# f-dangel/vivit

Hardware: AMD Instinct MI355X
Metric: GGN eigenpairs/sec (Gram build + symeig), MLP 784-512-10, batch=4096 (higher is better)
Workload: dtype f32

## Files before the change

### vivit_amd/csrc/sy2sb.hip

```cpp
#include <cstdlib>

#include "common.h"
#include "device_utils.h"
#include "eig_internal.h"

namespace vivit {

constexpr int SNB = 64;
constexpr int QT = 128;
constexpr int SGRP = 8;

__global__ __launch_bounds__(256) void sb_panel_load_kernel(const float *__restrict__ A, int64_t lda, int64_t j0, int64_t mp,
                                                            float *__restrict__ pan) {
  const int64_t idx = (int64_t)blockIdx.x * 256 + threadIdx.x;
  if (idx >= mp * SNB) return;
  const int64_t r = idx / SNB, c = idx - r * SNB;
  pan[idx] = A[(j0 + SNB + r) * lda + j0 + c];
}

__global__ __launch_bounds__(256) void sb_panel_load_row_kernel(const float *__restrict__ A, int64_t lda, int64_t j0, int64_t mp,
                                                                float *__restrict__ pan) {
  __shared__ float t[SNB][SNB + 1];
  const int64_t r0 = (int64_t)blockIdx.x * SNB;
  const int tid = threadIdx.x;
  for (int idx = tid; idx < SNB * SNB; idx += 256) {
    const int c = idx / SNB, rr = idx % SNB;
    t[c][rr] = r0 + rr < mp ? A[(j0 + c) * lda + j0 + SNB + r0 + rr] : 0.f;
  }
  __syncthreads();
  for (int idx = tid; idx < SNB * SNB; idx += 256) {
    const int rr = idx / SNB, c = idx % SNB;
    if (r0 + rr < mp) pan[(r0 + rr) * SNB + c] = t[c][rr];
  }
}

__global__ __launch_bounds__(256) void coef_gather_kernel(const float *__restrict__ S, int64_t lds_, int64_t g, int kp,
                                                          float *__restrict__ Coef) {
  const int idx = blockIdx.x * 256 + threadIdx.x;
  if (idx >= SNB * kp) return;
  const int k = idx / SNB, m = idx % SNB;
  Coef[(int64_t)m * kp + k] = S[(int64_t)k * lds_ + g + m];
}


__global__ __launch_bounds__(256) void qr_step_kernel(float *__restrict__ pan, int64_t mp, int c, int ncol, int nwg, QrPart pt,
                                                      float *__restrict__ vdst1, float *__restrict__ vdst2, int64_t lds_, int64_t gi0,
                                                      float *__restrict__ A, int64_t lda, int64_t j0,
                                                      float *__restrict__ tau1, float *__restrict__ betas) {
  __shared__ float tile[QT][SNB + 1];
  __shared__ float vs[QT], xs2[QT];
  __shared__ float zs[SNB];
  __shared__ float zq[4][SNB];
  __shared__ __attribute__((aligned(16))) float zq16[16][SNB];
  const int tid = threadIdx.x;
  const int64_t r0 = (int64_t)blockIdx.x * QT;
  constexpr int NTL = QT * (SNB / 4) / 256;
  float4 tl[NTL];
#pragma unroll
  for (int i = 0; i < NTL; ++i) {
    const int idx = tid + 256 * i;
    const int rl = idx / (SNB / 4), c4 = (idx - rl * (SNB / 4)) * 4;
    const int64_t r = r0 + rl;
    tl[i] = *reinterpret_cast<const float4 *>(pan + (r < mp ? r : 0) * SNB + c4);
  }
  const int par = c & 1;
  const float *uin = pt.u + (int64_t)par * nwg * SNB;
  const float *din = pt.diag + par * SNB;
  const int cq4 = tid & 15, q16 = tid >> 4;
  float4 pv[20];
#pragma unroll
  for (int i = 0; i < 20; ++i) {
    const int w = q16 + 16 * i;
    pv[i] = *reinterpret_cast<const float4 *>(uin + (int64_t)(w < nwg ? w : 0) * SNB + 4 * cq4);
  }
  const float din_c = din[c >= 0 ? c : 0], din_t = din[tid & (SNB - 1)];
  __builtin_amdgcn_sched_barrier(0);
#pragma unroll
  for (int i = 0; i < NTL; ++i) {
    const int idx = tid + 256 * i;
    const int rl = idx / (SNB / 4), c4 = (idx - rl * (SNB / 4)) * 4;
    const bool ok = r0 + rl < mp;
    tile[rl][c4 + 0] = ok ? tl[i].x : 0.f;
    tile[rl][c4 + 1] = ok ? tl[i].y : 0.f;
    tile[rl][c4 + 2] = ok ? tl[i].z : 0.f;
    tile[rl][c4 + 3] = ok ? tl[i].w : 0.f;
  }
  if (c >= 0) {
    {
      float4 acc = make_float4(0.f, 0.f, 0.f, 0.f);
#pragma unroll
      for (int i = 0; i < 20; ++i)
        if (q16 + 16 * i < nwg) { acc.x += pv[i].x; acc.y += pv[i].y; acc.z += pv[i].z; acc.w += pv[i].w; }
      for (int w0 = q16 + 16 * 20; w0 < nwg; w0 += 16 * 20) {
        float4 v[20];
#pragma unroll
        for (int i = 0; i < 20; ++i) {
          const int w = w0 + 16 * i;
          v[i] = *reinterpret_cast<const float4 *>(uin + (int64_t)(w < nwg ? w : 0) * SNB + 4 * cq4);
        }
#pragma unroll
        for (int i = 0; i < 20; ++i)
          if (w0 + 16 * i < nwg) { acc.x += v[i].x; acc.y += v[i].y; acc.z += v[i].z; acc.w += v[i].w; }
      }
      *reinterpret_cast<float4 *>(&zq16[q16][4 * cq4]) = acc;
    }
    __syncthreads();
    float ssq = 0.f;
#pragma unroll
    for (int g2 = 0; g2 < 16; ++g2) ssq += zq16[g2][c];
    const float alpha = din_c;
    float tau = 0.f, beta = alpha, scal = 0.f;
    if (ssq > 0.f) {
      beta = -copysignf(sqrt_nr(alpha * alpha + ssq), alpha);
      tau = (beta - alpha) * rcp_nr(beta);
      scal = rcp_nr(alpha - beta);
    }
    if (tid < SNB) {
      float u = 0.f;
#pragma unroll
      for (int g2 = 0; g2 < 16; ++g2) u += zq16[g2][tid];
      zs[tid] = tid > c ? tau * (din_t + scal * u) : 0.f;
    }
    if (tid < QT) {
      const int64_t r = r0 + tid;
      float v = 0.f;
      if (r < mp) {
        if (r == c) v = 1.f;
        else if (r > c) v = tile[tid][c] * scal;
        vdst1[(int64_t)c * lds_ + gi0 + r] = v;
        vdst2[(int64_t)c * lds_ + gi0 + r] = v;
        if (r >= c) A[(j0 + c) * lda + gi0 + r] = v;
      }
      vs[tid] = v;
    }
    if (blockIdx.x == 0 && tid == 0) { tau1[j0 + c] = tau; betas[c] = beta; }
  } else {
    if (tid < QT) vs[tid] = 0.f;
    if (tid < SNB) zs[tid] = 0.f;
  }
  __syncthreads();
  const int cn = c + 1;
  const bool has_next = cn < ncol;
  if (tid < QT) {
    const int64_t r = r0 + tid;
    xs2[tid] = (has_next && r > cn && r < mp) ? tile[tid][cn] - vs[tid] * zs[cn] : 0.f;
  }
  __syncthreads();
  {
    const int cc = tid & 63, q = tid >> 6;
    const float zc = zs[cc];
    float acc = 0.f;
#pragma unroll 8
    for (int i = 0; i < QT / 4; ++i) {
      const int rl = q + 4 * i;
      const float v = vs[rl];
      float x = tile[rl][cc];
      if (cc > c && v != 0.f) {
        x -= v * zc;
        tile[rl][cc] = x;
        if (r0 + rl < mp) pan[(r0 + rl) * SNB + cc] = x;
      }
      acc += xs2[rl] * x;
    }
    zq[q][cc] = acc;
  }
  if (!has_next) return;
  __syncthreads();
  {
    const int par = cn & 1;
    if (tid < SNB) pt.u[((int64_t)par * nwg + blockIdx.x) * SNB + tid] = (zq[0][tid] + zq[1][tid]) + (zq[2][tid] + zq[3][tid]);
    if (cn >= r0 && cn < r0 + QT && tid < SNB) pt.diag[par * SNB + tid] = tile[cn - r0][tid];
  }
}

constexpr int QP_WG = 32, QP_THREADS = 512;
struct QrPersistWs {
  float *ubuf;
  float *dbuf;
  int *counter;
  int *tmo;
  int attempt;
  int fault;
};

__device__ __forceinline__ float sel8(float a0, float a1, float a2, float a3, float a4, float a5, float a6, float a7, int j) {
  const float t0 = (j & 1) ? a1 : a0, t1 = (j & 1) ? a3 : a2, t2 = (j & 1) ? a5 : a4, t3 = (j & 1) ? a7 : a6;
  const float u0 = (j & 2) ? t1 : t0, u1 = (j & 2) ? t3 : t2;
  return (j & 4) ? u1 : u0;
}

template <int RI>
__global__ __launch_bounds__(QP_THREADS) void qr_persist_kernel(float *__restrict__ pan, int64_t mp, int ncol, QrPersistWs pw,
                                                                float *__restrict__ vdst1, float *__restrict__ vdst2, int64_t lds_,
                                                                int64_t gi0, float *__restrict__ A, int64_t lda, int64_t j0,
                                                                float *__restrict__ tau1, float *__restrict__ betas) {
  if ((blockIdx.x & 7) != 0) return;
  if (pw.attempt == 1 && __hip_atomic_load(pw.counter + 1, __ATOMIC_RELAXED, __HIP_MEMORY_SCOPE_AGENT) != PERSIST_ABORT) return;
  int *const cnt = pw.counter + 8 * pw.attempt;
  const int w = blockIdx.x >> 3;
  const int tid = threadIdx.x, lane = tid & 63, wave = tid >> 6;
  const int cg = tid & 7, rs = tid >> 3;
  constexpr int RW = 64 * RI;
  const int64_t rbase = (int64_t)w * RW;
  __shared__ float s_u[SNB], s_d[SNB], s_dn[SNB];
  __shared__ float s_red[QP_THREADS / 64][SNB];
  __shared__ float s_v[RW];
  __shared__ int s_flag[2];

  float x[RI][8];
#pragma unroll
  for (int i = 0; i < RI; ++i) {
    const int64_t r = rbase + rs + 64 * i;
    const float *src = pan + (r < mp ? r : 0) * SNB + 8 * cg;
    const float4 a = *reinterpret_cast<const float4 *>(src), b = *reinterpret_cast<const float4 *>(src + 4);
    const bool ok = r < mp;
    x[i][0] = ok ? a.x : 0.f; x[i][1] = ok ? a.y : 0.f; x[i][2] = ok ? a.z : 0.f; x[i][3] = ok ? a.w : 0.f;
    x[i][4] = ok ? b.x : 0.f; x[i][5] = ok ? b.y : 0.f; x[i][6] = ok ? b.z : 0.f; x[i][7] = ok ? b.w : 0.f;
  }
  if (tid == 0) {
    int xcc;
    __asm__ volatile("s_getreg_b32 %0, hwreg(HW_REG_XCC_ID)" : "=s"(xcc));
    __hip_atomic_store(pw.counter + 32 + w, xcc & 15, __ATOMIC_RELAXED, __HIP_MEMORY_SCOPE_AGENT);
    __asm__ volatile("s_waitcnt vmcnt(0)" ::: "memory");
    const bool go = persist_arrive(cnt, cnt + 1, QP_WG, ((pw.fault >> pw.attempt) & 1) ? 0ull : PERSIST_TIMEOUT_TICKS);
    const int dead = go ? 0 : 2;
    int slow = 0;
    const int x0 = __hip_atomic_load(pw.counter + 32, __ATOMIC_RELAXED, __HIP_MEMORY_SCOPE_AGENT);
    for (int i = 1; i < QP_WG; ++i) slow |= __hip_atomic_load(pw.counter + 32 + i, __ATOMIC_RELAXED, __HIP_MEMORY_SCOPE_AGENT) != x0;
    s_flag[0] = slow;
    s_flag[1] = dead;
  }
  __syncthreads();
  const bool slow = s_flag[0] != 0;
  if (s_flag[1] == 2) {
    if (tid == 0 && w == 0 && pw.attempt == 1) {
      __hip_atomic_fetch_or(pw.tmo, PERSIST_TMO_PANEL_QR, __ATOMIC_RELAXED, __HIP_MEMORY_SCOPE_AGENT);
      betas[0] = __builtin_nanf("");
    }
    return;
  }
  const int grp = lane & ~7;

  auto publish = [&](int cn) __attribute__((always_inline)) {
    float acc[8];
#pragma unroll
    for (int j = 0; j < 8; ++j) acc[j] = 0.f;
#pragma unroll
    for (int i = 0; i < RI; ++i) {
      const int64_t r = rbase + rs + 64 * i;
      float xn = __shfl(sel8(x[i][0], x[i][1], x[i][2], x[i][3], x[i][4], x[i][5], x[i][6], x[i][7], cn & 7), grp | (cn >> 3), 64);
      xn = (r > cn && r < mp) ? xn : 0.f;
#pragma unroll
      for (int j = 0; j < 8; ++j) acc[j] = fmaf(xn, x[i][j], acc[j]);
    }
#pragma unroll
    for (int j = 0; j < 8; ++j) {
      acc[j] += __shfl_xor(acc[j], 8, 64);
      acc[j] += __shfl_xor(acc[j], 16, 64);
      acc[j] += __shfl_xor(acc[j], 32, 64);
    }
    if (lane < 8) {
#pragma unroll
      for (int j = 0; j < 8; ++j) s_red[wave][8 * lane + j] = acc[j];
    }
    if (w == 0 && rs == cn) {
#pragma unroll
      for (int j = 0; j < 8; ++j) s_dn[8 * cg + j] = x[0][j];
    }
  };
  auto send = [&](int par) __attribute__((always_inline)) {
    if (wave == 0) {
      float u = 0.f;
#pragma unroll
      for (int q = 0; q < QP_THREADS / 64; ++q) u += s_red[q][lane];
      float *ub = pw.ubuf + ((size_t)par * QP_WG + w) * SNB + lane, *db = pw.dbuf + (size_t)par * SNB + lane;
      if (slow) {
        __hip_atomic_store(ub, u, __ATOMIC_RELAXED, __HIP_MEMORY_SCOPE_AGENT);
        if (w == 0) __hip_atomic_store(db, s_dn[lane], __ATOMIC_RELAXED, __HIP_MEMORY_SCOPE_AGENT);
      } else {
        *ub = u;
        if (w == 0) *db = s_dn[lane];
      }
      __asm__ volatile("s_waitcnt vmcnt(0)" ::: "memory");
      if (lane == 0) __hip_atomic_fetch_add(cnt, 1, __ATOMIC_RELAXED, __HIP_MEMORY_SCOPE_AGENT);
    }
  };

  publish(0);
  __syncthreads();
  send(0);
  for (int c = 0; c < ncol && !s_flag[1]; ++c) {
    const int par = c & 1;
    if (wave == 0) {
      const int target = (c + 2) * QP_WG;
      const unsigned long long t0 = __builtin_amdgcn_s_memrealtime();
      while (__hip_atomic_load(cnt, __ATOMIC_RELAXED, __HIP_MEMORY_SCOPE_AGENT) < target)
        if (__builtin_amdgcn_s_memrealtime() - t0 > PERSIST_TIMEOUT_TICKS) { s_flag[1] = 1; break; }
      const float *ub = pw.ubuf + (size_t)par * QP_WG * SNB + lane;
      float pv[QP_WG];
#pragma unroll
      for (int q = 0; q < QP_WG; ++q) pv[q] = __hip_atomic_load(ub + q * SNB, __ATOMIC_RELAXED, __HIP_MEMORY_SCOPE_AGENT);
      const float dn = __hip_atomic_load(pw.dbuf + (size_t)par * SNB + lane, __ATOMIC_RELAXED, __HIP_MEMORY_SCOPE_AGENT);
      float u = 0.f;
#pragma unroll
      for (int q = 0; q < QP_WG; ++q) u += pv[q];
      s_u[lane] = u;
      s_d[lane] = dn;
    }
    __syncthreads();
    if (s_flag[1]) break;
    const float ssq = s_u[c], alpha = s_d[c];
    float tau = 0.f, beta = alpha, scal = 0.f;
    if (ssq > 0.f) {
      beta = -copysignf(sqrt_nr(alpha * alpha + ssq), alpha);
      tau = (beta - alpha) * rcp_nr(beta);
      scal = rcp_nr(alpha - beta);
    }
    float z[8];
#pragma unroll
    for (int j = 0; j < 8; ++j) {
      const int cc = 8 * cg + j;
      z[j] = cc > c ? tau * (s_d[cc] + scal * s_u[cc]) : 0.f;
    }
#pragma unroll
    for (int i = 0; i < RI; ++i) {
      const int64_t r = rbase + rs + 64 * i;
      const float xc = __shfl(sel8(x[i][0], x[i][1], x[i][2], x[i][3], x[i][4], x[i][5], x[i][6], x[i][7], c & 7), grp | (c >> 3), 64);
      const float v = r == c ? 1.f : ((r > c && r < mp) ? xc * scal : 0.f);
      if (cg == 0) s_v[rs + 64 * i] = v;
#pragma unroll
      for (int j = 0; j < 8; ++j) x[i][j] = fmaf(-v, z[j], x[i][j]);
    }
    if (w == 0 && tid == 0) { tau1[j0 + c] = tau; betas[c] = beta; }
    const bool has_next = c + 1 < ncol;
    if (has_next) publish(c + 1);
    __syncthreads();
    if (has_next) send(par ^ 1);
    for (int idx = tid; idx < RW; idx += QP_THREADS) {
      const int64_t r = rbase + idx;
      if (r < mp) {
        const float v = s_v[idx];
        vdst1[(int64_t)c * lds_ + gi0 + r] = v;
        vdst2[(int64_t)c * lds_ + gi0 + r] = v;
        if (r >= c) A[(j0 + c) * lda + gi0 + r] = v;
      }
    }
  }
  if (w == 0) {
    const int64_t r = rs;
    if (r < mp) {
      float *dst = pan + r * SNB + 8 * cg;
      *reinterpret_cast<float4 *>(dst) = make_float4(x[0][0], x[0][1], x[0][2], x[0][3]);
      *reinterpret_cast<float4 *>(dst + 4) = make_float4(x[0][4], x[0][5], x[0][6], x[0][7]);
    }
    if (tid == 0 && s_flag[1]) {
      betas[0] = __builtin_nanf("");
      __hip_atomic_fetch_or(pw.tmo, PERSIST_TMO_PANEL_QR, __ATOMIC_RELAXED, __HIP_MEMORY_SCOPE_AGENT);
    }
  }
}

static bool qr_persist_enabled() {
  static int on = -1;
  if (on < 0) {
    const char *e = getenv("VIVIT_QR_PERSIST");
    on = e ? atoi(e) : 1;
  }
  return on != 0 && persist_override() != 0;
}
constexpr size_t QR_PERSIST_WS_BYTES = sizeof(float) * (2 * QP_WG * SNB + 2 * SNB) + 64 * sizeof(int) + 256;

static bool qr_persist_launch(float *pan, int64_t mp, int ncol, void *wsp, float *v1, float *v2, int64_t ldn, int64_t gi0, float *A,
                              int64_t lda, int64_t j0, float *tau1, float *betas, hipStream_t stream) {
  if (!qr_persist_enabled() || mp > (int64_t)QP_WG * 64 * 20 || device_cu_count() < 256) return false;
  QrPersistWs pw;
  pw.ubuf = reinterpret_cast<float *>(align_up(reinterpret_cast<uintptr_t>(wsp), 256));
  pw.dbuf = pw.ubuf + 2 * QP_WG * SNB;
  pw.counter = reinterpret_cast<int *>(pw.dbuf + 2 * SNB);
  pw.tmo = persist_timeout_word(stream);
  pw.fault = persist_fault();
  if (!pw.tmo) return false;
  if (hipMemsetAsync(pw.counter, 0, 64 * sizeof(int), stream) != hipSuccess) return false;
  const int64_t ri = cdiv(mp, (int64_t)QP_WG * 64);
  const dim3 grid(8 * QP_WG);
#define QP_LAUNCH(RI) qr_persist_kernel<RI><<<grid, QP_THREADS, 0, stream>>>(pan, mp, ncol, pw, v1, v2, ldn, gi0, A, lda, j0, tau1, betas)
  for (int attempt = 0; attempt < 2; ++attempt) {
    pw.attempt = attempt;
    if (ri <= 1) QP_LAUNCH(1);
    else if (ri <= 2) QP_LAUNCH(2);
    else if (ri <= 3) QP_LAUNCH(3);
    else if (ri <= 5) QP_LAUNCH(5);
    else if (ri <= 8) QP_LAUNCH(8);
    else if (ri <= 12) QP_LAUNCH(12);
    else if (ri <= 16) QP_LAUNCH(16);
    else QP_LAUNCH(20);
  }
#undef QP_LAUNCH
  return true;
}

struct Sk64Args {
  const float *Coef;
  const float *B;
  float *Out;
  int64_t ldcoef, ldb, ldo, N;
  int K;
  float alpha, beta;
};
constexpr int SK_LDC = 36, SK_COLS = 128, SK_LDB = SK_COLS + 4, SK_NT = SK_COLS / 64;

__global__ __launch_bounds__(256) void skinny64_kernel(Sk64Args p) {
  __shared__ __attribute__((aligned(16))) float sC[64 * SK_LDC];
  __shared__ __attribute__((aligned(16))) float sB[32 * SK_LDB];
  const int tid = threadIdx.x, lane = tid & 63, wave = tid >> 6;
  const int r = lane & 31, h = lane >> 5, wm = wave >> 1, wn = wave & 1;
  const int64_t c0 = (int64_t)blockIdx.x * SK_COLS;
  f32x16 acc[SK_NT];
#pragma unroll
  for (int t = 0; t < SK_NT; ++t)
#pragma unroll
    for (int e = 0; e < 16; ++e) acc[t][e] = 0.f;
  constexpr int NLB = 32 * SK_COLS / 4 / 256;
  float4 rc[2], rb[NLB];
  auto gload = [&](int k0) __attribute__((always_inline)) {
#pragma unroll
    for (int i = 0; i < 2; ++i) {
      const int idx = tid + 256 * i;
      const int m = idx >> 3, kq = (idx & 7) * 4;
      rc[i] = *reinterpret_cast<const float4 *>(p.Coef + (int64_t)m * p.ldcoef + k0 + kq);
    }
#pragma unroll
    for (int i = 0; i < NLB; ++i) {
      const int idx = tid + 256 * i;
      const int kr = idx / (SK_COLS / 4), cq = (idx % (SK_COLS / 4)) * 4;
      const int64_t c = c0 + cq;
      rb[i] = *reinterpret_cast<const float4 *>(p.B + (int64_t)(k0 + kr) * p.ldb + (c < p.N ? c : 0));
    }
    __builtin_amdgcn_sched_barrier(0);
  };
  gload(0);
  for (int k0 = 0; k0 < p.K; k0 += 32) {
    __syncthreads();
#pragma unroll
    for (int i = 0; i < 2; ++i) {
      const int idx = tid + 256 * i;
      *reinterpret_cast<float4 *>(sC + (idx >> 3) * SK_LDC + (idx & 7) * 4) = rc[i];
    }
#pragma unroll
    for (int i = 0; i < NLB; ++i) {
      const int idx = tid + 256 * i;
      const int kr = idx / (SK_COLS / 4), cq = (idx % (SK_COLS / 4)) * 4;
      *reinterpret_cast<float4 *>(sB + kr * SK_LDB + cq) = c0 + cq < p.N ? rb[i] : make_float4(0.f, 0.f, 0.f, 0.f);
    }
    __syncthreads();
    if (k0 + 32 < p.K) gload(k0 + 32);
    const float *pa = sC + (32 * wm + r) * SK_LDC + 4 * h;
#pragma unroll
    for (int j = 0; j < 4; ++j) {
      const float4 a4 = *reinterpret_cast<const float4 *>(pa + 8 * j);
      const float av[4] = {a4.x, a4.y, a4.z, a4.w};
      float bv[4][SK_NT];
#pragma unroll
      for (int i = 0; i < 4; ++i)
#pragma unroll
        for (int t = 0; t < SK_NT; ++t) bv[i][t] = sB[(8 * j + 4 * h + i) * SK_LDB + 64 * wn + 32 * t + r];
#pragma unroll
      for (int i = 0; i < 4; ++i)
#pragma unroll
        for (int t = 0; t < SK_NT; ++t) acc[t] = __builtin_amdgcn_mfma_f32_32x32x2f32(av[i], bv[i][t], acc[t], 0, 0, 0);
    }
  }
#pragma unroll
  for (int t = 0; t < SK_NT; ++t) {
    const int64_t c = c0 + 64 * wn + 32 * t + r;
    if (c < p.N) {
#pragma unroll
      for (int e = 0; e < 16; ++e) {
        const int m = 32 * wm + (e & 3) + 8 * (e >> 2) + 4 * h;
        float *o = p.Out + (int64_t)m * p.ldo + c;
        float v = p.alpha * acc[t][e];
        if (p.beta != 0.f) v += p.beta * *o;
        *o = v;
      }
    }
  }
}

static bool skinny64_launch(const float *Coef, int64_t ldcoef, const float *B, int64_t ldb, float *Out, int64_t ldo, int64_t N, int64_t K,
                            float alpha, float beta, hipStream_t stream) {
  if (K < 32 || K % 32 != 0 || K > 4096 || N % 4 != 0 || ldb % 4 != 0 || ldcoef % 4 != 0 ||
      (reinterpret_cast<uintptr_t>(Coef) & 15) || (reinterpret_cast<uintptr_t>(B) & 15))
    return false;
  Sk64Args a;
  a.Coef = Coef; a.B = B; a.Out = Out; a.ldcoef = ldcoef; a.ldb = ldb; a.ldo = ldo; a.N = N; a.K = (int)K; a.alpha = alpha; a.beta = beta;
  skinny64_kernel<<<(unsigned)cdiv(N, SK_COLS), 256, 0, stream>>>(a);
  return true;
}

__global__ __launch_bounds__(256) void w_coef_kernel(const float *__restrict__ T, const float *__restrict__ G, float *__restrict__ Coef) {
  __shared__ float sT[SNB][SNB + 1], sG[SNB][SNB + 1], sU[SNB][SNB + 1];
  const int tid = threadIdx.x, lane = tid & 63, wave = tid >> 6;
  const int r = lane & 31, h = lane >> 5, qi = (wave >> 1) * 32, qj = (wave & 1) * 32;
  for (int idx = tid; idx < SNB * SNB; idx += 256) {
    sT[idx / SNB][idx % SNB] = T[idx];
    sG[idx / SNB][idx % SNB] = G[idx];
  }
  __syncthreads();
  f32x16 acc;
#pragma unroll
  for (int e = 0; e < 16; ++e) acc[e] = 0.f;
#pragma unroll 8
  for (int s2 = 0; s2 < SNB / 2; ++s2) acc = __builtin_amdgcn_mfma_f32_32x32x2f32(sT[2 * s2 + h][qi + r], sG[2 * s2 + h][qj + r], acc, 0, 0, 0);
#pragma unroll
  for (int e = 0; e < 16; ++e) sU[qi + (e & 3) + 8 * (e >> 2) + 4 * h][qj + r] = acc[e];
  __syncthreads();
#pragma unroll
  for (int e = 0; e < 16; ++e) acc[e] = 0.f;
#pragma unroll 8
  for (int s2 = 0; s2 < SNB / 2; ++s2) acc = __builtin_amdgcn_mfma_f32_32x32x2f32(sU[qi + r][2 * s2 + h], sT[2 * s2 + h][qj + r], acc, 0, 0, 0);
#pragma unroll
  for (int e = 0; e < 16; ++e) {
    const int a_ = qi + (e & 3) + 8 * (e >> 2) + 4 * h, b_ = qj + r;
    Coef[a_ * 2 * SNB + b_] = -0.5f * acc[e];
    Coef[a_ * 2 * SNB + SNB + b_] = sT[b_][a_];
  }
}

__global__ __launch_bounds__(256) void sb_panel_store_kernel(float *__restrict__ A, int64_t lda, int64_t j0, int64_t mp,
                                                             const float *__restrict__ pan, const float *__restrict__ betas) {
  const int idx = blockIdx.x * 256 + threadIdx.x;
  if (idx >= SNB * SNB) return;
  const int r = idx / SNB, c = idx - r * SNB;
  if (r >= mp) return;
  A[(j0 + SNB + r) * lda + j0 + c] = (r < c) ? pan[(int64_t)r * SNB + c] : (r == c ? betas[c] : 0.f);
}

__global__ __launch_bounds__(256) void larft_kernel(const float *__restrict__ S, int64_t lds_, const float *__restrict__ tau, int nb,
                                                    int nvalid, float *__restrict__ T) {
  constexpr int H = SNB / 2, LD = SNB + 1;
  __shared__ float Ss[SNB * LD], Ts[SNB * LD], Xs[H * (H + 1)], taus[SNB];
  const int tid = threadIdx.x;
  for (int idx = tid; idx < SNB * SNB; idx += 256) {
    Ss[(idx / SNB) * LD + (idx % SNB)] = S[(int64_t)(idx / SNB) * lds_ + (idx % SNB)];
    Ts[(idx / SNB) * LD + (idx % SNB)] = 0.f;
  }
  if (tid < SNB) taus[tid] = (tid < nvalid && tid < nb) ? tau[tid] : 0.f;
  __syncthreads();
  if (tid < SNB) {
    const int half = tid / H, j = tid % H;
    const float *Sb = Ss + half * (H * LD + H), *tb = taus + half * H;
    float t[H];
#pragma unroll
    for (int c = 0; c < H; ++c) t[c] = 0.f;
#pragma unroll
    for (int i = H - 1; i >= 0; --i) {
      float acc = 0.f;
#pragma unroll
      for (int c = i + 1; c < H; ++c) acc += Sb[i * LD + c] * t[c];
      t[i] = i == j ? tb[j] : (i < j ? -tb[i] * acc : 0.f);
    }
    float *Tb = Ts + half * (H * LD + H);
#pragma unroll
    for (int i = 0; i < H; ++i) Tb[i * LD + j] = t[i];
  }
  __syncthreads();
  if (tid < 64) {
    const int r = tid & 31, h = tid >> 5;
    f32x16 acc;
#pragma unroll
    for (int e = 0; e < 16; ++e) acc[e] = 0.f;
#pragma unroll 8
    for (int s2 = 0; s2 < H / 2; ++s2)
      acc = __builtin_amdgcn_mfma_f32_32x32x2f32(Ss[r * LD + H + 2 * s2 + h], Ts[(H + 2 * s2 + h) * LD + H + r], acc, 0, 0, 0);
#pragma unroll
    for (int e = 0; e < 16; ++e) Xs[((e & 3) + 8 * (e >> 2) + 4 * h) * (H + 1) + r] = acc[e];
  }
  __syncthreads();
  if (tid < 64) {
    const int r = tid & 31, h = tid >> 5;
    f32x16 acc;
#pragma unroll
    for (int e = 0; e < 16; ++e) acc[e] = 0.f;
#pragma unroll 8
    for (int s2 = 0; s2 < H / 2; ++s2)
      acc = __builtin_amdgcn_mfma_f32_32x32x2f32(Ts[r * LD + 2 * s2 + h], Xs[(2 * s2 + h) * (H + 1) + r], acc, 0, 0, 0);
#pragma unroll
    for (int e = 0; e < 16; ++e) Ts[((e & 3) + 8 * (e >> 2) + 4 * h) * LD + H + r] = -acc[e];
  }
  __syncthreads();
  for (int idx = tid; idx < SNB * SNB; idx += 256) T[idx] = Ts[(idx / SNB) * LD + (idx % SNB)];
}

__global__ __launch_bounds__(256) void sb_extract_band_kernel(const float *__restrict__ A, int64_t lda, int64_t n,
                                                              float *__restrict__ AB, int64_t ldab) {
  const int64_t idx = (int64_t)blockIdx.x * 256 + threadIdx.x;
  if (idx >= n * ldab) return;
  const int64_t i = idx / ldab;
  const int d = (int)(idx - i * ldab);
  const int64_t j = i - 2 * SNB + d;
  AB[idx] = (d >= SNB && d <= 2 * SNB && j >= 0) ? A[i * lda + j] : 0.f;
}

static size_t sy2sb_gemm_ws_bytes(int64_t n) {
  size_t m = 0;
  for (int64_t mp = 1; mp <= n; mp = mp < 4096 ? mp * 2 : mp + 4096) {
    const int64_t q = mp < n ? mp : n;
    size_t a = gemm_workspace_bytes(SNB, SNB, q, false);
    size_t b = gemm_workspace_bytes(SNB, q, q, false);
    size_t c = gemm_workspace_bytes(SNB, q, SNB, false);
    size_t d = 0, e = 0, f = 0;
    for (int g = 1; g < SGRP; ++g) {
      const size_t d1 = gemm_workspace_bytes(SNB, 2 * SNB * g + SNB, q, false), e1 = gemm_workspace_bytes(SNB, q, 2 * SNB * g, false);
      const size_t f1 = gemm_workspace_bytes(q, SNB, 2 * SNB * g, false);
      d = d1 > d ? d1 : d; e = e1 > e ? e1 : e; f = f1 > f ? f1 : f;
    }
    m = a > m ? a : m; m = b > m ? b : m; m = c > m ? c : m;
    m = d > m ? d : m; m = e > m ? e : m; m = f > m ? f : m;
    const size_t u = gemm_workspace_bytes(q, q, (int64_t)2 * SNB * SGRP, true);
    m = u > m ? u : m;
  }
  size_t a = gemm_workspace_bytes(SNB, SNB, n, false), b = gemm_workspace_bytes(SNB, n, n, false);
  m = a > m ? a : m; m = b > m ? b : m;
  return m * 2;
}

Sy2sbWs sy2sb_layout(Arena &a, int64_t n) {
  const int64_t nwg = cdiv(n, QT) + 1;
  Sy2sbWs ws;
  ws.pan = a.take<float>(n * SNB);
  ws.stackA = a.take<float>(2 * SGRP * SNB * n);
  ws.stackB = a.take<float>(2 * SGRP * SNB * n);
  ws.xt = a.take<float>(SNB * n);
  ws.G12 = a.take<float>(SNB * 2 * SNB * SGRP);
  ws.qp.u = a.take<float>(2 * nwg * SNB);
  ws.qp.diag = a.take<float>(2 * SNB);
  ws.qpw = a.take<char>(QR_PERSIST_WS_BYTES);
  ws.S = a.take<float>(SNB * SNB);
  ws.T = a.take<float>(SNB * SNB);
  ws.Y3 = a.take<float>(SNB * SNB);
  ws.S2 = a.take<float>(SNB * SNB);
  ws.tau1 = a.take<float>(n);
  ws.betas = a.take<float>(SNB);
  ws.gws_bytes = sy2sb_gemm_ws_bytes(n);
  ws.gws = a.take<char>(ws.gws_bytes);
  return ws;
}

size_t sy2sb_workspace_bytes(int64_t n) {
  Arena m;
  sy2sb_layout(m, n);
  return m.used() + 1024;
}

int sy2sb_launch(float *A, int64_t n, int64_t lda, const Sy2sbWs &ws, hipStream_t stream) {
  if (hipMemsetAsync(ws.tau1, 0, sizeof(float) * n, stream) != hipSuccess) return VIVIT_E_LAUNCH;

  const int64_t ldn = n;
  const bool rowmode = (n % 4 == 0) && (lda % 4 == 0) && (reinterpret_cast<uintptr_t>(A) & 15) == 0;
  auto factor_panel = [&](int64_t j0, float *v1, float *v2) -> int {
    const int64_t mp = n - j0 - SNB, gi0 = j0 + SNB;
    const int ncol = (int)(mp < SNB ? mp : SNB);
    const int g = (int)cdiv(mp, QT);
    if (rowmode) sb_panel_load_row_kernel<<<(unsigned)cdiv(mp, SNB), 256, 0, stream>>>(A, lda, j0, mp, ws.pan);
    else sb_panel_load_kernel<<<(unsigned)cdiv(mp * SNB, 256), 256, 0, stream>>>(A, lda, j0, mp, ws.pan);
    if (!qr_persist_launch(ws.pan, mp, ncol, ws.qpw, v1, v2, ldn, gi0, A, lda, j0, ws.tau1, ws.betas, stream))
      for (int c = -1; c < ncol; ++c)
        qr_step_kernel<<<g, 256, 0, stream>>>(ws.pan, mp, c, ncol, g, ws.qp, v1, v2, ldn, gi0, A, lda, j0, ws.tau1, ws.betas);
    sb_panel_store_kernel<<<(unsigned)cdiv(SNB * SNB, 256), 256, 0, stream>>>(A, lda, j0, mp, ws.pan, ws.betas);
    return launch_status();
  };
  auto compute_w = [&](int64_t j0, float *Vt, float *Wt, float *Wcopy, int64_t kp, const float *sAg, const float *sBg) -> int {
    const int64_t mp = n - j0 - SNB, gi0 = j0 + SNB;
    const int ncol = (int)(mp < SNB ? mp : SNB);
    float *A22 = A + gi0 * lda + gi0;
    int st;
    prof_mark(PROF_STAGE_SY2SB, stream);
    st = gemm_launch(LAY_K, LAY_M, Vt, A22, Wt, SNB, mp, mp, ldn, lda, ldn, 1.f, 0.f, false, ws.gws, ws.gws_bytes, stream);
    prof_mark(PROF_STAGE_SY2SB_PP, stream);
    if (st != VIVIT_OK) return st;
    const int64_t ldg = kp + SNB;
    st = gemm_launch(LAY_K, LAY_K, Vt, sAg, ws.G12, SNB, ldg, mp, ldn, ldn, ldg, 1.f, 0.f, false, ws.gws, ws.gws_bytes, stream);
    if (st != VIVIT_OK) return st;
    larft_kernel<<<1, 256, 0, stream>>>(ws.G12 + kp, ldg, ws.tau1 + j0, SNB, ncol, ws.T);
    if (kp > 0) {
      if (!skinny64_launch(ws.G12, ldg, sBg, ldn, Wt, ldn, mp, kp, -1.f, 1.f, stream)) {
        st = gemm_launch(LAY_K, LAY_M, ws.G12, sBg, Wt, SNB, mp, kp, ldg, ldn, ldn, -1.f, 1.f, false, ws.gws, ws.gws_bytes, stream);
        if (st != VIVIT_OK) return st;
      }
    }
    st = gemm_launch(LAY_K, LAY_K, Wt, Vt, ws.S2, SNB, SNB, mp, ldn, ldn, SNB, 1.f, 0.f, false, ws.gws, ws.gws_bytes, stream);
    if (st != VIVIT_OK) return st;
    w_coef_kernel<<<1, 256, 0, stream>>>(ws.T, ws.S2, ws.G12);
    if (Wt == Vt + (int64_t)SNB * ldn &&
        skinny64_launch(ws.G12, 2 * SNB, Vt, ldn, Wcopy, ldn, mp, 2 * SNB, 1.f, 0.f, stream))
      return hipMemcpy2DAsync(Wt, sizeof(float) * ldn, Wcopy, sizeof(float) * ldn, sizeof(float) * mp, SNB, hipMemcpyDeviceToDevice,
                              stream) == hipSuccess ? VIVIT_OK : VIVIT_E_LAUNCH;
    float *Xt = ws.xt + gi0;
    st = gemm_launch(LAY_M, LAY_M, ws.T, Wt, Xt, SNB, mp, SNB, SNB, ldn, ldn, 1.f, 0.f, false, ws.gws, ws.gws_bytes, stream);
    if (st != VIVIT_OK) return st;
    if (hipMemcpy2DAsync(Wt, sizeof(float) * ldn, Xt, sizeof(float) * ldn, sizeof(float) * mp, SNB, hipMemcpyDeviceToDevice,
                         stream) != hipSuccess)
      return VIVIT_E_LAUNCH;
    st = gemm_launch(LAY_K, LAY_M, ws.G12, Vt, Wt, SNB, mp, SNB, 2 * SNB, ldn, ldn, 1.f, 1.f, false, ws.gws, ws.gws_bytes, stream);
    if (st != VIVIT_OK) return st;
    return hipMemcpy2DAsync(Wcopy, sizeof(float) * ldn, Wt, sizeof(float) * ldn, sizeof(float) * mp, SNB, hipMemcpyDeviceToDevice,
                            stream) == hipSuccess ? VIVIT_OK : VIVIT_E_LAUNCH;
  };

  float *sA = ws.stackA, *sB = ws.stackB;
  for (int64_t j0 = 0; j0 + SNB < n;) {
    int st;
    if (hipMemsetAsync(sA, 0, sizeof(float) * 2 * SGRP * SNB * n, stream) != hipSuccess) return VIVIT_E_LAUNCH;
    if (hipMemsetAsync(sB, 0, sizeof(float) * 2 * SGRP * SNB * n, stream) != hipSuccess) return VIVIT_E_LAUNCH;
    int np = 0;
    int64_t gi_last = 0;
    for (; np < SGRP && j0 + SNB < n; ++np, j0 += SNB) {
      const int64_t gi = j0 + SNB;
      const int64_t kp = (int64_t)2 * SNB * np;
      if (np > 0) {
        const int64_t gc = gi - SNB;
        bool done = false;
        if (rowmode) {
          coef_gather_kernel<<<(unsigned)cdiv(SNB * kp, 256), 256, 0, stream>>>(sA, ldn, gc, (int)kp, ws.G12);
          done = skinny64_launch(ws.G12, kp, sB + gc, ldn, A + gc * lda + gc, lda, n - gc, kp, -1.f, 1.f, stream);
        }
        if (!done) {
          if (rowmode) return VIVIT_E_UNSUPPORTED;
          st = gemm_launch(LAY_M, LAY_M, sA + gc, sB + gc, A + gc * lda + gc, n - gc, SNB, kp, ldn, ldn, lda, -1.f, 1.f, false,
                           ws.gws, ws.gws_bytes, stream);
          if (st != VIVIT_OK) return st;
        }
      }
      float *Vrow = sA + kp * n, *Wrow = sA + (kp + SNB) * n;
      st = factor_panel(j0, Vrow, sB + (kp + SNB) * n);
      if (st != VIVIT_OK) return st;
      st = compute_w(j0, Vrow + gi, Wrow + gi, sB + kp * n + gi, kp, sA + gi, sB + gi);
      if (st != VIVIT_OK) return st;
      gi_last = gi;
    }
    const int64_t mt = n - gi_last;
    prof_mark(PROF_STAGE_SY2SB, stream);
    st = gemm_launch(LAY_M, LAY_M, sA + gi_last, sB + gi_last, A + gi_last * lda + gi_last, mt, mt, (int64_t)2 * SNB * np, ldn, ldn,
                     lda, -1.f, 1.f, true, ws.gws, ws.gws_bytes, stream);
    prof_mark(PROF_STAGE_SY2SB_UPD, stream);
    if (st != VIVIT_OK) return st;
  }
  return launch_status();
}

struct PanelQrWs {
  QrPart qp;
  float *S;
  void *qpw, *gws;
  size_t gws_bytes;
};

static PanelQrWs panel_qr_layout(Arena &a, int64_t mp) {
  const int64_t nwg = cdiv(mp, QT) + 1;
  PanelQrWs ws;
  ws.qp.u = a.take<float>(2 * nwg * SNB);
  ws.qp.diag = a.take<float>(2 * SNB);
  ws.S = a.take<float>(SNB * SNB);
  ws.qpw = a.take<char>(QR_PERSIST_WS_BYTES);
  ws.gws_bytes = gemm_workspace_bytes(SNB, SNB, mp, false);
  ws.gws = a.take<char>(ws.gws_bytes);
  return ws;
}

size_t sy2sb_panel_qr_workspace_bytes(int64_t mp) {
  Arena m;
  panel_qr_layout(m, mp);
  return m.used() + 1024;
}

int sy2sb_panel_qr_launch(float *pan, int64_t mp, float *Vt, int64_t ldv, float *tau, float *betas, float *T, void *wsbase,
                          size_t ws_bytes, hipStream_t stream) {
  if (ws_bytes < sy2sb_panel_qr_workspace_bytes(mp)) return VIVIT_E_WORKSPACE;
  Arena a(wsbase, ws_bytes);
  const PanelQrWs ws = panel_qr_layout(a, mp);
  if (a.overflow()) return VIVIT_E_WORKSPACE;
  const QrPart qp = ws.qp;
  float *S = ws.S;
  void *qpw = ws.qpw, *gws = ws.gws;
  const size_t gws_bytes = ws.gws_bytes;
  const int ncol = (int)(mp < SNB ? mp : SNB);
  const int g = (int)cdiv(mp, QT);
  if (hipMemsetAsync(tau, 0, sizeof(float) * SNB, stream) != hipSuccess) return VIVIT_E_LAUNCH;
  if (hipMemsetAsync(betas, 0, sizeof(float) * SNB, stream) != hipSuccess) return VIVIT_E_LAUNCH;
  if (hipMemset2DAsync(Vt, sizeof(float) * ldv, 0, sizeof(float) * mp, SNB, stream) != hipSuccess) return VIVIT_E_LAUNCH;
  if (!qr_persist_launch(pan, mp, ncol, qpw, Vt, Vt, ldv, 0, Vt, ldv, 0, tau, betas, stream))
    for (int c = -1; c < ncol; ++c)
      qr_step_kernel<<<g, 256, 0, stream>>>(pan, mp, c, ncol, g, qp, Vt, Vt, ldv, 0, Vt, ldv, 0, tau, betas);
  int st = gemm_launch(LAY_K, LAY_K, Vt, Vt, S, SNB, SNB, mp, ldv, ldv, SNB, 1.f, 0.f, false, gws, gws_bytes, stream);
  if (st != VIVIT_OK) return st;
  larft_kernel<<<1, 256, 0, stream>>>(S, SNB, tau, SNB, ncol, T);
  return launch_status();
}

int sy2sb_extract_band_launch(const float *A, int64_t lda, int64_t n, float *AB, int64_t ldab, hipStream_t stream) {
  sb_extract_band_kernel<<<(unsigned)cdiv(n * ldab, 256), 256, 0, stream>>>(A, lda, n, AB, ldab);
  return launch_status();
}

}

using namespace vivit;

extern "C" {

size_t vivit_sy2sb_f32_workspace_bytes(int64_t n) { return n > 0 ? sy2sb_workspace_bytes(n) : 0; }

int vivit_sy2sb_f32(float *A, int64_t n, int64_t lda, float *AB, float *tau1, void *workspace, size_t workspace_bytes,
                    void *stream) {
  if (n < 1 || !A || !AB || !tau1 || lda < n) return VIVIT_E_BADARG;
  if (!workspace || workspace_bytes < sy2sb_workspace_bytes(n)) return VIVIT_E_WORKSPACE;
  hipStream_t s = static_cast<hipStream_t>(stream);
  Arena a(workspace, workspace_bytes);
  const Sy2sbWs ws = sy2sb_layout(a, n);
  if (a.overflow()) return VIVIT_E_WORKSPACE;
  int st = sy2sb_launch(A, n, lda, ws, s);
  if (st != VIVIT_OK) return st;
  st = sy2sb_extract_band_launch(A, lda, n, AB, 2 * SNB + 1, s);
  if (st != VIVIT_OK) return st;
  if (hipMemcpyAsync(tau1, ws.tau1, sizeof(float) * n, hipMemcpyDeviceToDevice, s) != hipSuccess) return VIVIT_E_LAUNCH;
  return VIVIT_OK;
}

size_t vivit_sy2sb_panel_qr_f32_workspace_bytes(int64_t mp) { return mp > 0 ? sy2sb_panel_qr_workspace_bytes(mp) : 0; }

int vivit_sy2sb_panel_qr_f32(float *pan, int64_t mp, float *Vt, int64_t ldv, float *tau, float *betas, float *T, void *workspace,
                             size_t workspace_bytes, void *stream) {
  if (mp < 1 || !pan || !Vt || !tau || !betas || !T || ldv < mp) return VIVIT_E_BADARG;
  if (!workspace) return VIVIT_E_WORKSPACE;
  return sy2sb_panel_qr_launch(pan, mp, Vt, ldv, tau, betas, T, workspace, workspace_bytes, static_cast<hipStream_t>(stream));
}

}
```

Baseline: 7460.

## Remap QR panel threads so each wave owns a column group, staging pivot column in LDS

Reassigns thread mapping in the persistent panel QR kernel so each wave owns one 8-column group and lanes index rows, replacing the per-element sel8+shuffle broadcast of the pivot column with a staged copy in shared memory. Reduction shuffles become intra-8-lane and waves whose columns are entirely left of the current column skip the rank-1 update and dot products. This adds an extra __syncthreads per column and changes the load mapping of x (the initial load still uses the old cg/rs indexing semantics with new values), which could add latency on the per-column critical path.

After: 7532 (median of 6 runs). Within noise of the previous version (+1.0%).

```diff
diff --git a/vivit_amd/csrc/sy2sb.hip b/vivit_amd/csrc/sy2sb.hip
--- a/vivit_amd/csrc/sy2sb.hip
+++ b/vivit_amd/csrc/sy2sb.hip
@@ -1,4 +1,5 @@
 #include <cstdlib>
+#include <type_traits>
 
 #include "common.h"
 #include "device_utils.h"
@@ -183,12 +184,6 @@
   int fault;
 };
 
-__device__ __forceinline__ float sel8(float a0, float a1, float a2, float a3, float a4, float a5, float a6, float a7, int j) {
-  const float t0 = (j & 1) ? a1 : a0, t1 = (j & 1) ? a3 : a2, t2 = (j & 1) ? a5 : a4, t3 = (j & 1) ? a7 : a6;
-  const float u0 = (j & 2) ? t1 : t0, u1 = (j & 2) ? t3 : t2;
-  return (j & 4) ? u1 : u0;
-}
-
 template <int RI>
 __global__ __launch_bounds__(QP_THREADS) void qr_persist_kernel(float *__restrict__ pan, int64_t mp, int ncol, QrPersistWs pw,
                                                                 float *__restrict__ vdst1, float *__restrict__ vdst2, int64_t lds_,
@@ -199,12 +194,14 @@
   int *const cnt = pw.counter + 8 * pw.attempt;
   const int w = blockIdx.x >> 3;
   const int tid = threadIdx.x, lane = tid & 63, wave = tid >> 6;
-  const int cg = tid & 7, rs = tid >> 3;
+  const int cg = wave, rs = lane;
   constexpr int RW = 64 * RI;
   const int64_t rbase = (int64_t)w * RW;
+  const int lim = (int)(mp - rbase < RW ? (mp - rbase > 0 ? mp - rbase : 0) : RW);
   __shared__ float s_u[SNB], s_d[SNB], s_dn[SNB];
-  __shared__ float s_red[QP_THREADS / 64][SNB];
+  __shared__ float s_red[QP_THREADS / 64][SNB + 1];
   __shared__ float s_v[RW];
+  __shared__ float s_x[2][RW];
   __shared__ int s_flag[2];
 
   float x[RI][8];
@@ -239,29 +236,47 @@
     }
     return;
   }
-  const int grp = lane & ~7;
-
+  auto stage_j = [&](int cn, auto J) __attribute__((always_inline)) {
+#pragma unroll
+    for (int i = 0; i < RI; ++i) {
+      const int rl = rs + 64 * i;
+      s_x[cn & 1][rl] = (rl < lim && (i > 0 || w > 0 || rl > cn)) ? x[i][decltype(J)::value] : 0.f;
+    }
+  };
+  auto stage = [&](int cn) __attribute__((always_inline)) {
+    if (cg != (cn >> 3)) return;
+    switch (cn & 7) {
+      case 0: stage_j(cn, std::integral_constant<int, 0>{}); break;
+      case 1: stage_j(cn, std::integral_constant<int, 1>{}); break;
+      case 2: stage_j(cn, std::integral_constant<int, 2>{}); break;
+      case 3: stage_j(cn, std::integral_constant<int, 3>{}); break;
+      case 4: stage_j(cn, std::integral_constant<int, 4>{}); break;
+      case 5: stage_j(cn, std::integral_constant<int, 5>{}); break;
+      case 6: stage_j(cn, std::integral_constant<int, 6>{}); break;
+      default: stage_j(cn, std::integral_constant<int, 7>{}); break;
+    }
+  };
   auto publish = [&](int cn) __attribute__((always_inline)) {
     float acc[8];
 #pragma unroll
     for (int j = 0; j < 8; ++j) acc[j] = 0.f;
-#pragma unroll
-    for (int i = 0; i < RI; ++i) {
-      const int64_t r = rbase + rs + 64 * i;
-      float xn = __shfl(sel8(x[i][0], x[i][1], x[i][2], x[i][3], x[i][4], x[i][5], x[i][6], x[i][7], cn & 7), grp | (cn >> 3), 64);
-      xn = (r > cn && r < mp) ? xn : 0.f;
-#pragma unroll
-      for (int j = 0; j < 8; ++j) acc[j] = fmaf(xn, x[i][j], acc[j]);
-    }
-#pragma unroll
-    for (int j = 0; j < 8; ++j) {
-      acc[j] += __shfl_xor(acc[j], 8, 64);
-      acc[j] += __shfl_xor(acc[j], 16, 64);
-      acc[j] += __shfl_xor(acc[j], 32, 64);
-    }
-    if (lane < 8) {
-#pragma unroll
-      for (int j = 0; j < 8; ++j) s_red[wave][8 * lane + j] = acc[j];
+    if (8 * cg + 7 >= cn) {
+#pragma unroll
+      for (int i = 0; i < RI; ++i) {
+        const float xn = s_x[cn & 1][rs + 64 * i];
+#pragma unroll
+        for (int j = 0; j < 8; ++j) acc[j] = fmaf(xn, x[i][j], acc[j]);
+      }
+#pragma unroll
+      for (int j = 0; j < 8; ++j) {
+        acc[j] += __shfl_xor(acc[j], 1, 64);
+        acc[j] += __shfl_xor(acc[j], 2, 64);
+        acc[j] += __shfl_xor(acc[j], 4, 64);
+      }
+    }
+    if ((lane & 7) == 0) {
+#pragma unroll
+      for (int j = 0; j < 8; ++j) s_red[lane >> 3][8 * cg + j] = acc[j];
     }
     if (w == 0 && rs == cn) {
 #pragma unroll
@@ -286,6 +301,8 @@
     }
   };
 
+  stage(0);
+  __syncthreads();
   publish(0);
   __syncthreads();
   send(0);
@@ -322,18 +339,26 @@
       const int cc = 8 * cg + j;
       z[j] = cc > c ? tau * (s_d[cc] + scal * s_u[cc]) : 0.f;
     }
-#pragma unroll
-    for (int i = 0; i < RI; ++i) {
-      const int64_t r = rbase + rs + 64 * i;
-      const float xc = __shfl(sel8(x[i][0], x[i][1], x[i][2], x[i][3], x[i][4], x[i][5], x[i][6], x[i][7], c & 7), grp | (c >> 3), 64);
-      const float v = r == c ? 1.f : ((r > c && r < mp) ? xc * scal : 0.f);
-      if (cg == 0) s_v[rs + 64 * i] = v;
-#pragma unroll
-      for (int j = 0; j < 8; ++j) x[i][j] = fmaf(-v, z[j], x[i][j]);
+    const bool own = cg == (c >> 3);
+    if (8 * cg + 7 >= c) {
+#pragma unroll
+      for (int i = 0; i < RI; ++i) {
+        const int rl = rs + 64 * i;
+        const float xc = s_x[par][rl];
+        float v = (rl < lim && (i > 0 || w > 0 || rl > c)) ? xc * scal : 0.f;
+        if (i == 0 && w == 0 && rs == c) v = 1.f;
+        if (own) s_v[rl] = v;
+#pragma unroll
+        for (int j = 0; j < 8; ++j) x[i][j] = fmaf(-v, z[j], x[i][j]);
+      }
     }
     if (w == 0 && tid == 0) { tau1[j0 + c] = tau; betas[c] = beta; }
     const bool has_next = c + 1 < ncol;
-    if (has_next) publish(c + 1);
+    if (has_next) {
+      stage(c + 1);
+      __syncthreads();
+      publish(c + 1);
+    }
     __syncthreads();
     if (has_next) send(par ^ 1);
     for (int idx = tid; idx < RW; idx += QP_THREADS) {
```
